# jkulhanek/viewformer

Hardware: NVIDIA H100
Metric: novel views/sec (128x128, 9-ctx) (higher is better)
Workload: dtype f32 encoder (bit-exact codes) + bf16 transformer/decoder

## Files before the change

viewformer_b200/csrc/vf_tc_gemm.cu:

```cuda
#include "vf_wgmma.cuh"
#include <stdlib.h>

namespace {
using namespace vftc;

constexpr int BLOCK_M = 128;
constexpr int ROW_BYTES = 128;
constexpr int A_STAGE_BYTES = BLOCK_M * ROW_BYTES;
constexpr int NUM_EPI_WARPS = 8;
constexpr int NUM_MMA_THREADS = 32 * NUM_EPI_WARPS;
constexpr int NUM_THREADS = NUM_MMA_THREADS + 128;

struct TcParams {
    CUtensorMap tmA, tmB;
    int conv;
    int M, Ncols;
    int num_k_blocks;
    int batch2;
    int tiles_m, tiles_n, total_tiles;
    int a_bm1, a_bm2, b_bm1, b_bm2;
    int TW, TH, TN, tiles_x, tiles_y, OH, OW, Nimg, cin_blocks, bk_elems;
    int tap_dy[9], tap_dx[9], tap_coff[9];
    int gemm_koff;
    int causal_block, causal_skip_n;
    float alpha;
    const float* bias;
    int bias_mode, act;
    const float* residual;
    float* C_f32;
    __nv_bfloat16* C_bf16;
    long long ldc, c_sb1, c_sb2;
    int vec_ok;
    int halo;
    double* gn_sums;
    int gn_groups, gn_cpg, gn_rows_per_img;
    int exact;
    int exact_kc;
    int exact_clog;
    int exact_kpp;
    int exact_lo_b;
    const float2* norm_mr;
    const float* norm_gamma;
    const float* norm_beta;
    int norm_groups, norm_cpg, norm_swish;
};

constexpr float EXACT_LO_SCALE = 1.0f / 2048.0f;

struct TileInfo {
    int m0, n0, b1, b2, img0, oy0, ox0, nkb;
    bool skip;
};

__device__ __forceinline__ TileInfo decode_tile(const TcParams& p, int t, int block_n) {
    TileInfo ti;
    const int n_tile = t % p.tiles_n;
    const int r = t / p.tiles_n;
    const int m_tile = r % p.tiles_m;
    const int bz = r / p.tiles_m;
    ti.b1 = bz / p.batch2;
    ti.b2 = bz % p.batch2;
    ti.m0 = m_tile * BLOCK_M;
    ti.n0 = n_tile * block_n;
    ti.nkb = p.num_k_blocks;
    ti.skip = false;
    if (p.causal_block > 0) {
        const int lim = ((ti.m0 + BLOCK_M - 1) / p.causal_block + 1) * p.causal_block;
        if (p.causal_skip_n) {
            ti.skip = ti.n0 >= lim;
        } else {
            const int kb = (lim + p.bk_elems - 1) / p.bk_elems;
            if (kb < ti.nkb) ti.nkb = kb;
        }
    }
    ti.img0 = ti.oy0 = ti.ox0 = 0;
    if (p.conv) {
        const int tx = m_tile % p.tiles_x;
        const int q = m_tile / p.tiles_x;
        ti.img0 = (q / p.tiles_y) * p.TN;
        ti.oy0 = (q % p.tiles_y) * p.TH;
        ti.ox0 = tx * p.TW;
    }
    return ti;
}

constexpr int HALO_BYTES = 23552;
constexpr int HALO_SLOTS = 6;
__host__ __device__ constexpr int operand_bytes(int stages, int stage_bytes, int b_stage_bytes) {
    return stages * stage_bytes > 2 * HALO_BYTES + HALO_SLOTS * b_stage_bytes ? stages * stage_bytes
                                                                               : 2 * HALO_BYTES + HALO_SLOTS * b_stage_bytes;
}
constexpr int MAX_STAGES = 8;
template <int kBlockN, int kStages>
__host__ __device__ constexpr int tc_smem_bytes() {
    return operand_bytes(kStages, A_STAGE_BYTES + kBlockN * ROW_BYTES, kBlockN * ROW_BYTES) +
           NUM_EPI_WARPS * 32 * (kBlockN / 2 + 4) * 4  + 1024  + 8 * (2 * MAX_STAGES + 4) ;
}

__device__ __forceinline__ void normalise_halo(const TcParams& p, uint8_t* tile, int cb, int img, int oy0, int ox0, int tid) {
    const int rows = (p.TW + 2) * (p.TH + 2);
    for (int idx = tid; idx < rows * 8; idx += NUM_MMA_THREADS) {
        const int r = idx >> 3, pc = idx & 7;
        const int py = r / (p.TW + 2), px = r - py * (p.TW + 2);
        const int iy = oy0 - 1 + py, ix = ox0 - 1 + px;
        if (iy < 0 || iy >= p.OH || ix < 0 || ix >= p.OW) continue;
        const int c0 = cb * 64 + ((pc ^ (r & 7)) << 3);
        uint4* ptr = reinterpret_cast<uint4*>(tile + r * ROW_BYTES + pc * 16);
        const uint4 v = *ptr;
        uint32_t w[4] = {v.x, v.y, v.z, v.w};
#pragma unroll
        for (int k = 0; k < 4; ++k) {
            const int c = c0 + 2 * k;
            const float2 ma = __ldg(p.norm_mr + (img * p.norm_groups + c / p.norm_cpg));
            const float2 mb = __ldg(p.norm_mr + (img * p.norm_groups + (c + 1) / p.norm_cpg));
            const float sa = ma.y * __ldg(p.norm_gamma + c), sb = mb.y * __ldg(p.norm_gamma + c + 1);
            float a = __uint_as_float(w[k] << 16), b = __uint_as_float(w[k] & 0xffff0000u);
            a = fmaf(a, sa, __ldg(p.norm_beta + c) - ma.x * sa);
            b = fmaf(b, sb, __ldg(p.norm_beta + c + 1) - mb.x * sb);
            if (p.norm_swish == 1) {
                a = __fdividef(a, 1.0f + __expf(-a));
                b = __fdividef(b, 1.0f + __expf(-b));
            }
            __nv_bfloat162 o = __floats2bfloat162_rn(a, b);
            w[k] = *reinterpret_cast<uint32_t*>(&o);
            if (p.norm_swish == 2) {
                uint32_t h, th;
                asm("mul.rn.bf16x2 %0, %1, %2;" : "=r"(h) : "r"(w[k]), "r"(0x3f003f00u));
                asm("tanh.approx.bf16x2 %0, %1;" : "=r"(th) : "r"(h));
                asm("fma.rn.bf16x2 %0, %1, %2, %1;" : "=r"(w[k]) : "r"(h), "r"(th));
            }
        }
        *ptr = make_uint4(w[0], w[1], w[2], w[3]);
    }
}

template <int kBlockN, int kStages, WgKind kKind>
__global__ void __launch_bounds__(NUM_THREADS, 1) tc_gemm_kernel(const __grid_constant__ TcParams p) {
    constexpr int B_STAGE_BYTES = kBlockN * ROW_BYTES;
    constexpr int STAGE_BYTES = A_STAGE_BYTES + B_STAGE_BYTES;
    constexpr int K_STEPS = 4;
    constexpr int HALF_N = kBlockN / 2;
    constexpr int STG_LD = HALF_N + 4;
    constexpr int STG_BYTES = NUM_EPI_WARPS * 32 * STG_LD * 4;
    constexpr int NACC = kBlockN / 2;
    constexpr bool kExact = kKind == F16;

    extern __shared__ uint8_t smem_raw[];
    uint8_t* smem = reinterpret_cast<uint8_t*>((reinterpret_cast<uintptr_t>(smem_raw) + 1023) & ~(uintptr_t)1023);
    constexpr int OPER_BYTES = operand_bytes(kStages, STAGE_BYTES, B_STAGE_BYTES);
    float* staging = reinterpret_cast<float*>(smem + OPER_BYTES);
    uint64_t* full_bar = reinterpret_cast<uint64_t*>(smem + OPER_BYTES + STG_BYTES);
    uint64_t* empty_bar = full_bar + MAX_STAGES;
    uint64_t* a_full_bar = empty_bar + MAX_STAGES;
    uint64_t* a_empty_bar = a_full_bar + 2;
    constexpr int NG = kStages;
    constexpr int NGH = HALO_SLOTS;
    uint8_t* halo_b_base = smem + 2 * HALO_BYTES;

    const int warp = threadIdx.x >> 5;
    const int lane = threadIdx.x & 31;

    if (threadIdx.x == 0) {
        prefetch_tmap(&p.tmA);
        prefetch_tmap(&p.tmB);
        for (int s = 0; s < MAX_STAGES; ++s) {
            mbar_init(&full_bar[s], 1);
            mbar_init(&empty_bar[s], NUM_MMA_THREADS);
        }
        for (int a = 0; a < 2; ++a) {
            mbar_init(&a_full_bar[a], 1);
            mbar_init(&a_empty_bar[a], NUM_MMA_THREADS);
        }
        mbar_fence_init();
    }
    __syncthreads();

    if (warp >= NUM_EPI_WARPS) {
        setmaxnreg_dec<40>();
        if (warp == NUM_EPI_WARPS && elect_one()) {
            int stage = 0;
            uint32_t phase = 0;
            int ab = 0;
            uint32_t aphase = 0;
            for (int t = blockIdx.x; t < p.total_tiles; t += gridDim.x) {
                const TileInfo ti = decode_tile(p, t, kBlockN);
                if (ti.skip) continue;
                if (p.halo) {
                    const uint32_t halo_bytes = (uint32_t)((p.TW + 2) * (p.TH + 2)) * ROW_BYTES;
                    const int nkb = 9 * p.cin_blocks;
                    int tap = 0, cb = 0;
                    for (int kb = 0; kb < nkb; ++kb) {
                        mbar_wait(&empty_bar[stage], phase ^ 1, "vf_tc_gemm producer");
                        mbar_expect_tx(&full_bar[stage], (uint32_t)B_STAGE_BYTES);
                        if (tap == 0) {
                            mbar_wait(&a_empty_bar[ab], aphase ^ 1, "vf_tc_gemm producer(halo)");
                            mbar_expect_tx(&a_full_bar[ab], halo_bytes);
                            tma_load_4d(smem + ab * HALO_BYTES, &p.tmA, &a_full_bar[ab], cb * p.bk_elems, ti.ox0 - 1, ti.oy0 - 1, ti.img0);
                            if (++ab == 2) { ab = 0; aphase ^= 1; }
                        }
                        tma_load_4d(halo_b_base + stage * B_STAGE_BYTES, &p.tmB, &full_bar[stage], (tap * p.cin_blocks + cb) * p.bk_elems,
                                    ti.n0, 0, 0);
                        if (++tap == 9) { tap = 0; ++cb; }
                        if (++stage == NGH) { stage = 0; phase ^= 1; }
                    }
                    continue;
                }
                for (int kb = 0; kb < ti.nkb; ++kb) {
                    mbar_wait(&empty_bar[stage], phase ^ 1, "vf_tc_gemm producer");
                    mbar_expect_tx(&full_bar[stage], (uint32_t)STAGE_BYTES);
                    uint8_t* sa = smem + stage * STAGE_BYTES;
                    uint8_t* sb = sa + A_STAGE_BYTES;
                    int kcoord_b = kb * p.bk_elems;
                    if (p.conv) {
                        int kbr = kb, a_half = 0;
                        if (p.exact) {
                            const int j = kb / p.exact_kpp;
                            kbr = kb - j * p.exact_kpp;
                            a_half = (j == 0) ? p.exact_clog : 0;
                            const int tap_ = kbr / p.cin_blocks, cb_ = kbr - tap_ * p.cin_blocks;
                            kcoord_b = ((tap_ * 2 + (j == 1 ? 1 : 0)) * p.cin_blocks + cb_) * p.bk_elems;
                        }
                        const int tap = kbr / p.cin_blocks;
                        const int cb = kbr - tap * p.cin_blocks;
                        tma_load_4d(sa, &p.tmA, &full_bar[stage], a_half + p.tap_coff[tap] + cb * p.bk_elems, ti.ox0 + p.tap_dx[tap],
                                    ti.oy0 + p.tap_dy[tap], ti.img0);
                    } else {
                        int kcoord_a = kb * p.bk_elems;
                        if (p.exact) {
                            const int j = kb / p.exact_kpp, kbr = kb - j * p.exact_kpp;
                            kcoord_a = (j == 0 ? p.exact_clog : 0) + kbr * p.bk_elems;
                            kcoord_b = (j == 1 ? p.exact_lo_b : 0) + kbr * p.bk_elems;
                        }
                        if (p.gemm_koff) kcoord_a += p.tap_coff[ti.b1];
                        tma_load_4d(sa, &p.tmA, &full_bar[stage], kcoord_a, ti.m0, ti.b2 * p.a_bm2, ti.b1 * p.a_bm1);
                    }
                    tma_load_4d(sb, &p.tmB, &full_bar[stage], kcoord_b, ti.n0, ti.b2 * p.b_bm2, ti.b1 * p.b_bm1);
                    if (++stage == NG) { stage = 0; phase ^= 1; }
                }
            }
        }
        return;
    }

    setmaxnreg_inc<232>();
    const int wg = warp >> 2;
    const int quarter = warp & 3;
    const int col_half = warp >> 2;
    float* stg = staging + warp * (32 * STG_LD);
    int stage = 0, ab = 0;
    uint32_t phase = 0, aphase = 0;

    auto to_staging = [&](const float (&v)[NACC], float sc) {
        const int r_lo = 64 * wg + 16 * (warp & 3) + (lane >> 2);
#pragma unroll
        for (int j = 0; j < NACC / 4; ++j) {
#pragma unroll
            for (int h = 0; h < 2; ++h) {
                const int r = r_lo + 8 * h, c = 8 * j + 2 * (lane & 3);
                float* dst = staging + ((c / HALF_N) * 4 + (r >> 5)) * (32 * STG_LD) + (r & 31) * STG_LD + (c % HALF_N);
                *reinterpret_cast<float2*>(dst) = make_float2(v[4 * j + 2 * h] * sc, v[4 * j + 2 * h + 1] * sc);
            }
        }
    };

    for (int t = blockIdx.x; t < p.total_tiles; t += gridDim.x) {
        const TileInfo ti = decode_tile(p, t, kBlockN);
        if (ti.skip) continue;

        float acc[NACC];
        float csum[kExact ? NACC : 1];
        auto k_loop = [&]() {
            const int nkb = p.halo ? 9 * p.cin_blocks : ti.nkb;
            const int nsmall = p.exact ? 2 * p.exact_kpp / p.exact_kc : 0;
            int prev_stage = -1, prev_halo = -1, in_chunk = 0, ck = 0, tap = 0;
            bool fresh = true;
            uint32_t a_base = 0;
            const uint32_t pitch = (uint32_t)(p.TW + 2);
            auto retire_prev = [&]() {
                if (prev_stage >= 0) mbar_arrive(&empty_bar[prev_stage]);
                if (prev_halo >= 0) mbar_arrive(&a_empty_bar[prev_halo]);
                prev_stage = prev_halo = -1;
            };
#pragma unroll 1
            for (int kb = 0; kb < nkb; ++kb) {
                uint64_t adesc, bdesc;
                const int this_halo = (p.halo && tap == 8) ? ab : -1;
                if (p.halo) {
                    if (tap == 0) {
                        mbar_wait(&a_full_bar[ab], aphase, "vf_tc_gemm mma(halo)");
                        a_base = smem_u32(smem + ab * HALO_BYTES);
                        if (!kExact && p.norm_mr) {
                            normalise_halo(p, smem + ab * HALO_BYTES, kb / 9, ti.img0, ti.oy0, ti.ox0, threadIdx.x);
                            fence_async_smem();
                            named_sync(1, NUM_MMA_THREADS);
                        }
                    }
                    mbar_wait(&full_bar[stage], phase, "vf_tc_gemm mma");
                    const uint32_t a_addr = a_base + ((uint32_t)(tap / 3) * pitch + (uint32_t)(tap % 3) + (uint32_t)(8 * wg) * pitch) * ROW_BYTES;
                    adesc = sw128_desc(a_addr, pitch * ROW_BYTES);
                    bdesc = sw128_desc(smem_u32(halo_b_base + stage * B_STAGE_BYTES));
                } else {
                    mbar_wait(&full_bar[stage], phase, "vf_tc_gemm mma");
                    const uint32_t sa = smem_u32(smem + stage * STAGE_BYTES);
                    adesc = sw128_desc(sa + (uint32_t)(wg * 64 * ROW_BYTES));
                    bdesc = sw128_desc(sa + A_STAGE_BYTES);
                }
                wgmma_fence();
#pragma unroll
                for (int k = 0; k < K_STEPS; ++k)
                    wgmma_ss<kBlockN, kKind>(acc, adesc + (uint64_t)(2 * k), bdesc + (uint64_t)(2 * k), (fresh && k == 0) ? 0u : 1u);
                wgmma_commit();
                fresh = false;
                wgmma_wait<1>();
                retire_prev();
                prev_stage = stage;
                prev_halo = this_halo;
                if (p.halo) {
                    if (++stage == NGH) { stage = 0; phase ^= 1; }
                    if (++tap == 9) { tap = 0; if (++ab == 2) { ab = 0; aphase ^= 1; } }
                } else {
                    if (++stage == NG) { stage = 0; phase ^= 1; }
                }
                if (kExact && ++in_chunk == p.exact_kc) {
                    in_chunk = 0;
                    wgmma_wait<0>();
                    reg_fence(acc);
                    const float sc = (ck < nsmall ? EXACT_LO_SCALE : 1.0f) * p.alpha;
                    if (ck == 0) {
#pragma unroll
                        for (int i = 0; i < NACC; ++i) csum[i] = acc[i] * sc;
                    } else {
#pragma unroll
                        for (int i = 0; i < NACC; ++i) csum[i] = fmaf(acc[i], sc, csum[i]);
                    }
                    ++ck;
                    fresh = true;
                }
            }
            wgmma_wait<0>();
            reg_fence(acc);
            retire_prev();
        };
        if constexpr (kExact) k_loop();

        const int row = quarter * 32 + lane;
        long long my_off;
        int my_ok, gm;
        if (p.conv) {
            const int lx = row % p.TW;
            const int q = row / p.TW;
            const int ly = q % p.TH;
            const int ln = q / p.TH;
            const int img = ti.img0 + ln, oy = ti.oy0 + ly, ox = ti.ox0 + lx;
            my_ok = (img < p.Nimg) && (oy < p.OH) && (ox < p.OW);
            gm = (img * p.OH + oy) * p.OW + ox;
            my_off = (long long)gm * p.ldc;
        } else {
            gm = ti.m0 + row;
            my_ok = gm < p.M;
            my_off = (long long)ti.b1 * p.c_sb1 + (long long)ti.b2 * p.c_sb2 + (long long)gm * p.ldc;
        }
        const float bias_m = (p.bias_mode == VF_BIAS_M && my_ok) ? __ldg(p.bias + gm) : 0.f;

        constexpr int VPR = HALF_N / 4;
        constexpr int RPI = 32 / VPR;
        constexpr int ITERS = 32 / RPI;
        const int r_sub = lane / VPR;
        const int c_ln = (lane % VPR) * 4;
        const int n_ln = ti.n0 + col_half * HALF_N + c_ln;
        const bool fast = p.vec_ok && (ti.n0 + kBlockN <= p.Ncols);
        auto residual_at = [&](int i) {
            const int rr = i * RPI + r_sub;
            const int ok = __shfl_sync(0xffffffffu, my_ok, rr);
            const long long off_row = __shfl_sync(0xffffffffu, my_off, rr);
            const long long o = ok ? off_row + n_ln : (long long)n_ln;
            return __ldg(reinterpret_cast<const float4*>(p.residual + o));
        };
        float4 resv[kExact ? 1 : ITERS];
        if (!kExact && fast && p.residual) {
#pragma unroll
            for (int i = 0; i < ITERS; ++i) resv[i] = residual_at(i);
        }
        float4 bias4 = make_float4(0.f, 0.f, 0.f, 0.f);
        if (fast && p.bias_mode == VF_BIAS_N) bias4 = __ldg(reinterpret_cast<const float4*>(p.bias + n_ln));

        if constexpr (!kExact) k_loop();
        named_sync(1, NUM_MMA_THREADS);
        if constexpr (kExact) to_staging(csum, 1.0f);
        else to_staging(acc, p.alpha);
        named_sync(1, NUM_MMA_THREADS);

        if (fast) {
            float gs = 0.f, gq = 0.f;
#pragma unroll
            for (int i = 0; i < ITERS; ++i) {
                const int rr = i * RPI + r_sub;
                const int ok = __shfl_sync(0xffffffffu, my_ok, rr);
                const long long off_row = __shfl_sync(0xffffffffu, my_off, rr);
                const float bm = __shfl_sync(0xffffffffu, bias_m, rr);
                float4 v = *reinterpret_cast<const float4*>(stg + rr * STG_LD + c_ln);
                if (p.bias_mode == VF_BIAS_N) { v.x += bias4.x; v.y += bias4.y; v.z += bias4.z; v.w += bias4.w; }
                else { v.x += bm; v.y += bm; v.z += bm; v.w += bm; }
                if (p.act == VF_ACT_GELU_ERF) { v.x = vf_gelu_erf(v.x); v.y = vf_gelu_erf(v.y); v.z = vf_gelu_erf(v.z); v.w = vf_gelu_erf(v.w); }
                if (p.residual) {
                    const float4 r = kExact ? residual_at(i) : resv[i];
                    v.x += r.x; v.y += r.y; v.z += r.z; v.w += r.w;
                }
                if (ok) {
                    gs += (v.x + v.y) + (v.z + v.w);
                    gq += (v.x * v.x + v.y * v.y) + (v.z * v.z + v.w * v.w);
                    const long long off = off_row + n_ln;
                    if (p.C_f32) *reinterpret_cast<float4*>(p.C_f32 + off) = v;
                    if (p.C_bf16) {
                        __nv_bfloat162 lo = __floats2bfloat162_rn(v.x, v.y), hi = __floats2bfloat162_rn(v.z, v.w);
                        uint2 u;
                        u.x = *reinterpret_cast<uint32_t*>(&lo);
                        u.y = *reinterpret_cast<uint32_t*>(&hi);
                        *reinterpret_cast<uint2*>(p.C_bf16 + off) = u;
                    }
                }
            }
            if (p.gn_sums) {
                const unsigned okmask = __ballot_sync(0xffffffffu, my_ok);
#pragma unroll
                for (int o = VPR; o < 32; o <<= 1) {
                    gs += __shfl_xor_sync(0xffffffffu, gs, o);
                    gq += __shfl_xor_sync(0xffffffffu, gq, o);
                }
                const int lpg = p.gn_cpg >> 2;
                for (int o = 1; o < lpg; o <<= 1) {
                    gs += __shfl_xor_sync(0xffffffffu, gs, o);
                    gq += __shfl_xor_sync(0xffffffffu, gq, o);
                }
                const int gm_first = __shfl_sync(0xffffffffu, gm, okmask ? (__ffs(okmask) - 1) : 0);
                if (okmask && r_sub == 0 && (lane % lpg) == 0) {
                    const long long slot = ((long long)(gm_first / p.gn_rows_per_img) * p.gn_groups + n_ln / p.gn_cpg) * 2;
                    atomicAdd(p.gn_sums + slot, (double)gs);
                    atomicAdd(p.gn_sums + slot + 1, (double)gq);
                }
            }
        } else {
#pragma unroll 1
            for (int rr = 0; rr < 32; ++rr) {
                const int ok = __shfl_sync(0xffffffffu, my_ok, rr);
                const long long off_row = __shfl_sync(0xffffffffu, my_off, rr);
                const float bm = __shfl_sync(0xffffffffu, bias_m, rr);
                if (!ok) continue;
                for (int c = lane; c < HALF_N; c += 32) {
                    const int n = ti.n0 + col_half * HALF_N + c;
                    if (n >= p.Ncols) continue;
                    float x = stg[rr * STG_LD + c];
                    x += (p.bias_mode == VF_BIAS_N) ? __ldg(p.bias + n) : bm;
                    if (p.act == VF_ACT_GELU_ERF) x = vf_gelu_erf(x);
                    const long long off = off_row + n;
                    if (p.residual) x += __ldg(p.residual + off);
                    if (p.C_f32) p.C_f32[off] = x;
                    if (p.C_bf16) p.C_bf16[off] = __float2bfloat16(x);
                }
            }
        }
    }
}

int make_tmap(CUtensorMap* tm, int dtype, const void* base, const uint64_t dims[4], const uint64_t strides_bytes[3],
              const uint32_t box[4]) {
    EncodeTiledFn fn = encode_fn();
    if (!fn) { vf_set_error("vf_tc_gemm: cuTensorMapEncodeTiled unavailable"); return VF_ERR_CUDA; }
    cuuint64_t gdim[4] = {dims[0], dims[1], dims[2], dims[3]};
    cuuint64_t gstr[3] = {strides_bytes[0], strides_bytes[1], strides_bytes[2]};
    cuuint32_t bx[4] = {box[0], box[1], box[2], box[3]};
    cuuint32_t es[4] = {1, 1, 1, 1};
    CUresult r = fn(tm, dtype == VF_BF16 ? CU_TENSOR_MAP_DATA_TYPE_BFLOAT16 : CU_TENSOR_MAP_DATA_TYPE_FLOAT32, 4,
                    const_cast<void*>(base), gdim, gstr, bx, es, CU_TENSOR_MAP_INTERLEAVE_NONE, CU_TENSOR_MAP_SWIZZLE_128B,
                    CU_TENSOR_MAP_L2_PROMOTION_L2_256B, CU_TENSOR_MAP_FLOAT_OOB_FILL_NONE);
    if (r != CUDA_SUCCESS) {
        vf_set_error("vf_tc_gemm: cuTensorMapEncodeTiled failed (%d): dims=[%llu,%llu,%llu,%llu] strides=[%llu,%llu,%llu] box=[%u,%u,%u,%u]",
                     (int)r, (unsigned long long)dims[0], (unsigned long long)dims[1], (unsigned long long)dims[2],
                     (unsigned long long)dims[3], (unsigned long long)strides_bytes[0], (unsigned long long)strides_bytes[1],
                     (unsigned long long)strides_bytes[2], box[0], box[1], box[2], box[3]);
        return VF_ERR_CUDA;
    }
    return VF_OK;
}

template <int kBlockN, int kStages, WgKind kKind>
int launch(const TcParams& prm, dim3 grid, cudaStream_t st) {
    constexpr int smem = tc_smem_bytes<kBlockN, kStages>();
    static_assert(kStages <= MAX_STAGES, "ring depth");
    static_assert(smem <= 232448, "shared memory budget");
    static vf_per_device_flag configured_pd;
    bool& configured = configured_pd.current();
    if (!configured) {
        cudaError_t e = cudaFuncSetAttribute(tc_gemm_kernel<kBlockN, kStages, kKind>, cudaFuncAttributeMaxDynamicSharedMemorySize, smem);
        if (e != cudaSuccess) { vf_set_error("vf_tc_gemm: cudaFuncSetAttribute: %s", cudaGetErrorString(e)); return VF_ERR_CUDA; }
        configured = true;
    }
    tc_gemm_kernel<kBlockN, kStages, kKind><<<grid, NUM_THREADS, smem, st>>>(prm);
    VF_CHECK_LAUNCH("vf_tc_gemm");
    return VF_OK;
}

template <int kBlockN, int kStages>
int launch_kind(const TcParams& prm, WgKind kind, dim3 grid, cudaStream_t st) {
    if (kind == TF32) return launch<kBlockN, kStages, TF32>(prm, grid, st);
    if (kind == F16) return launch<kBlockN, kStages, F16>(prm, grid, st);
    return launch<kBlockN, kStages, BF16>(prm, grid, st);
}

}

extern "C" int vf_tc_gemm(const vf_tc_gemm_t* q, vf_stream_t s) {
    VF_CHECK_ARG(q && q->A && q->B, "vf_tc_gemm: null operand");
    VF_CHECK_ARG(q->C_f32 || q->C_bf16, "vf_tc_gemm: no output");
    VF_CHECK_ARG(q->ab_dtype == VF_BF16 || q->ab_dtype == VF_F32 || q->ab_dtype == VF_F16X2, "vf_tc_gemm: bad dtype");
    const bool exact = q->ab_dtype == VF_F16X2;
    if (exact) {
        VF_CHECK_ARG(q->C_f32 && !q->C_bf16 && !q->norm_mean_rstd && q->causal_block == 0,
                     "vf_tc_gemm: VF_F16X2 (exact split-fp16) operands need an fp32 output and no causal / fused-norm options");
        if (q->conv) VF_CHECK_ARG(q->Ctot % 2 == 0 && q->alpha == 1.0f, "vf_tc_gemm: exact conv needs [hi | lo] channels and alpha = 1");
        else VF_CHECK_ARG(q->K % 64 == 0 && q->exact_lo_a >= q->K && q->exact_lo_b >= q->K && q->exact_lo_a % 8 == 0 && q->exact_lo_b % 8 == 0,
                          "vf_tc_gemm: exact GEMM needs K %% 64 == 0 and lo-half offsets >= K (K=%d lo_a=%lld lo_b=%lld)", q->K,
                          (long long)q->exact_lo_a, (long long)q->exact_lo_b);
    }
    VF_CHECK_ARG(q->bias_mode == VF_BIAS_NONE || q->bias, "vf_tc_gemm: bias pointer missing");
    VF_CHECK_ARG(!q->norm_mean_rstd || q->conv, "vf_tc_gemm: fused input GroupNorm is a convolution option");
    const bool tf32 = q->ab_dtype == VF_F32;
    const int tm_dtype = tf32 ? VF_F32 : VF_BF16;
    const int es = tf32 ? 4 : 2;
    const int bk = ROW_BYTES / es;

    TcParams prm;
    memset(&prm, 0, sizeof(prm));
    prm.conv = q->conv;
    prm.Ncols = q->Ncols;
    prm.bk_elems = bk;
    prm.alpha = q->alpha;
    prm.bias = q->bias;
    prm.bias_mode = q->bias_mode;
    prm.act = q->act;
    prm.residual = q->residual;
    prm.C_f32 = q->C_f32;
    prm.C_bf16 = reinterpret_cast<__nv_bfloat16*>(q->C_bf16);
    prm.ldc = q->ldc;
    prm.causal_block = q->causal_block;
    prm.causal_skip_n = q->causal_skip_n;

    const int block_n = (q->Ncols > 64) ? 128 : 64;
    const int b_box_rows = block_n;
    dim3 grid;
    int rc;
    if (q->conv) {
        VF_CHECK_ARG(q->ntaps >= 1 && q->ntaps <= 9, "vf_tc_gemm: ntaps");
        VF_CHECK_ARG(q->Cin % bk == 0 && q->Ctot % (16 / es) == 0, "vf_tc_gemm: conv Cin=%d must be a multiple of %d", q->Cin, bk);
        VF_CHECK_ARG(q->causal_block == 0, "vf_tc_gemm: causal with conv");
        int TW = q->OW >= 16 ? 16 : (q->OW >= 8 ? 8 : (q->OW >= 4 ? 4 : (q->OW >= 2 ? 2 : 1)));
        int TH = 128 / TW;
        if (TH > q->OH) { TH = 1; while (TH * 2 <= q->OH) TH *= 2; }
        int TN = 128 / (TW * TH);
        bool halo = !exact && q->ntaps == 9 && q->Ctot == q->Cin && q->OH == q->H && q->OW == q->W && q->OH >= 16 && q->OW >= 8;
        for (int t = 0; halo && t < 9; ++t) halo = q->tap_dy[t] == t / 3 - 1 && q->tap_dx[t] == t % 3 - 1 && q->tap_coff[t] == 0;
        if (halo) { TW = 8; TH = 16; TN = 1; }
        prm.halo = halo ? 1 : 0;
        if (q->norm_mean_rstd) {
            VF_CHECK_ARG(halo && q->ab_dtype == VF_BF16 && q->H >= 32 && q->Ncols % 128 == 0 && q->Cin % 64 == 0,
                         "vf_tc_gemm: fused input GroupNorm needs a 3x3 stride-1 bf16 conv on a map >= 32 rows (Cin %% 64 == 0, Cout %% 128 == 0)");
            VF_CHECK_ARG(q->norm_gamma && q->norm_beta && q->norm_groups > 0 && q->Cin % q->norm_groups == 0,
                         "vf_tc_gemm: fused input GroupNorm needs gamma, beta and a group count dividing Cin");
            prm.norm_mr = reinterpret_cast<const float2*>(q->norm_mean_rstd);
            prm.norm_gamma = q->norm_gamma;
            prm.norm_beta = q->norm_beta;
            prm.norm_groups = q->norm_groups;
            prm.norm_cpg = q->Cin / q->norm_groups;
            prm.norm_swish = q->norm_swish;
        }
        VF_CHECK_ARG(TW * TH * TN == 128 && TN <= 256, "vf_tc_gemm: cannot tile %dx%d output", q->OH, q->OW);
        prm.TW = TW; prm.TH = TH; prm.TN = TN;
        prm.tiles_x = (q->OW + TW - 1) / TW;
        prm.tiles_y = (q->OH + TH - 1) / TH;
        prm.OH = q->OH; prm.OW = q->OW; prm.Nimg = q->N;
        prm.cin_blocks = q->Cin / bk;
        prm.num_k_blocks = q->ntaps * prm.cin_blocks;
        if (exact) {
            prm.exact = 1;
            prm.exact_kpp = prm.num_k_blocks;
            prm.exact_clog = q->Ctot / 2;
            prm.exact_kc = (prm.num_k_blocks % 3 == 0) ? 3 : 1;
            prm.num_k_blocks *= 3;
        }
        prm.M = q->N * q->OH * q->OW;
        prm.batch2 = 1;
        for (int t = 0; t < q->ntaps; ++t) { prm.tap_dy[t] = q->tap_dy[t]; prm.tap_dx[t] = q->tap_dx[t]; prm.tap_coff[t] = q->tap_coff[t]; }
        const uint64_t dimsA[4] = {(uint64_t)q->Ctot, (uint64_t)q->W, (uint64_t)q->H, (uint64_t)q->N};
        const uint64_t strA[3] = {(uint64_t)q->Ctot * es, (uint64_t)q->W * q->Ctot * es, (uint64_t)q->H * q->W * q->Ctot * es};
        const uint32_t boxA[4] = {(uint32_t)bk, (uint32_t)(halo ? TW + 2 : TW), (uint32_t)(halo ? TH + 2 : TH), (uint32_t)TN};
        if ((rc = make_tmap(&prm.tmA, tm_dtype, q->A, dimsA, strA, boxA)) != VF_OK) return rc;
        const uint64_t Ktot = (uint64_t)q->ntaps * q->Cin * (exact ? 2 : 1);
        const uint64_t dimsB[4] = {Ktot, (uint64_t)q->Ncols, 1, 1};
        const uint64_t strB[3] = {Ktot * es, Ktot * es * q->Ncols, Ktot * es * q->Ncols};
        const uint32_t boxB[4] = {(uint32_t)bk, (uint32_t)b_box_rows, 1, 1};
        if ((rc = make_tmap(&prm.tmB, tm_dtype, q->B, dimsB, strB, boxB)) != VF_OK) return rc;
        const int ntiles_img = (q->N + TN - 1) / TN;
        grid = dim3(prm.tiles_x * prm.tiles_y * ntiles_img, (q->Ncols + block_n - 1) / block_n, 1);
    } else {
        VF_CHECK_ARG(q->M > 0 && q->Ncols > 0 && q->K > 0 && q->batch1 > 0 && q->batch2 > 0, "vf_tc_gemm: bad shape");
        VF_CHECK_ARG((q->lda * es) % 16 == 0 && (q->ldb * es) % 16 == 0, "vf_tc_gemm: row strides must be 16-byte multiples");
        VF_CHECK_ARG((q->a_sb1 * es) % 16 == 0 && (q->a_sb2 * es) % 16 == 0 && (q->b_sb1 * es) % 16 == 0 && (q->b_sb2 * es) % 16 == 0,
                     "vf_tc_gemm: batch strides must be 16-byte multiples");
        prm.M = q->M;
        prm.batch2 = q->batch2;
        prm.num_k_blocks = (q->K + bk - 1) / bk;
        if (exact) {
            prm.exact = 1;
            prm.exact_kpp = prm.num_k_blocks;
            prm.exact_clog = (int)q->exact_lo_a;
            prm.exact_lo_b = (int)q->exact_lo_b;
            prm.exact_kc = prm.exact_kpp % 4 == 0 ? 4 : (prm.exact_kpp % 3 == 0 ? 3 : (prm.exact_kpp % 2 == 0 ? 2 : 1));
            prm.num_k_blocks *= 3;
        }
        prm.c_sb1 = q->c_sb1; prm.c_sb2 = q->c_sb2;
        long long max_koff = 0;
        if (q->ntaps > 0) {
            VF_CHECK_ARG(q->ntaps == q->batch1 && q->ntaps <= 9, "vf_tc_gemm: gemm K offsets need ntaps == batch1 <= 9");
            prm.gemm_koff = 1;
            for (int t = 0; t < q->ntaps; ++t) {
                VF_CHECK_ARG(q->tap_coff[t] >= 0 && q->tap_coff[t] % 8 == 0, "vf_tc_gemm: K offsets must be non-negative multiples of 8 (16-byte TMA box starts)");
                prm.tap_coff[t] = q->tap_coff[t];
                if (q->tap_coff[t] > max_koff) max_koff = q->tap_coff[t];
            }
        }
        prm.a_bm1 = (q->batch1 > 1 && q->a_sb1 != 0) ? 1 : 0;
        prm.a_bm2 = (q->batch2 > 1 && q->a_sb2 != 0) ? 1 : 0;
        prm.b_bm1 = (q->batch1 > 1 && q->b_sb1 != 0) ? 1 : 0;
        prm.b_bm2 = (q->batch2 > 1 && q->b_sb2 != 0) ? 1 : 0;
        const uint64_t fbA = (uint64_t)q->lda * es * (uint64_t)q->M, fbB = (uint64_t)q->ldb * es * (uint64_t)q->Ncols;
        const uint64_t dimsA[4] = {(uint64_t)((exact ? q->exact_lo_a + q->K : q->K) + max_koff), (uint64_t)q->M, prm.a_bm2 ? (uint64_t)q->batch2 : 1, prm.a_bm1 ? (uint64_t)q->batch1 : 1};
        const uint64_t strA[3] = {(uint64_t)q->lda * es, prm.a_bm2 ? (uint64_t)q->a_sb2 * es : fbA, prm.a_bm1 ? (uint64_t)q->a_sb1 * es : fbA};
        const uint32_t boxA[4] = {(uint32_t)bk, (uint32_t)BLOCK_M, 1, 1};
        if ((rc = make_tmap(&prm.tmA, tm_dtype, q->A, dimsA, strA, boxA)) != VF_OK) return rc;
        const uint64_t dimsB[4] = {(uint64_t)(exact ? q->exact_lo_b + q->K : q->K), (uint64_t)q->Ncols, prm.b_bm2 ? (uint64_t)q->batch2 : 1, prm.b_bm1 ? (uint64_t)q->batch1 : 1};
        const uint64_t strB[3] = {(uint64_t)q->ldb * es, prm.b_bm2 ? (uint64_t)q->b_sb2 * es : fbB, prm.b_bm1 ? (uint64_t)q->b_sb1 * es : fbB};
        const uint32_t boxB[4] = {(uint32_t)bk, (uint32_t)b_box_rows, 1, 1};
        if ((rc = make_tmap(&prm.tmB, tm_dtype, q->B, dimsB, strB, boxB)) != VF_OK) return rc;
        VF_CHECK_ARG(q->causal_block == 0 || (q->causal_block % bk == 0 || bk % q->causal_block == 0), "vf_tc_gemm: causal block");
        grid = dim3((q->M + BLOCK_M - 1) / BLOCK_M, (q->Ncols + block_n - 1) / block_n, q->batch1 * q->batch2);
    }
    prm.tiles_m = (int)grid.x;
    prm.tiles_n = (int)grid.y;
    const long long total = (long long)prm.tiles_m * grid.y * grid.z;
    VF_CHECK_ARG(total > 0 && total < (1ll << 31), "vf_tc_gemm: tile count out of range");
    prm.total_tiles = (int)total;
    static int num_sms = 0;
    if (num_sms == 0) {
        int dev = 0;
        cudaGetDevice(&dev);
        if (cudaDeviceGetAttribute(&num_sms, cudaDevAttrMultiProcessorCount, dev) != cudaSuccess || num_sms <= 0) num_sms = 132;
    }
    const dim3 pgrid((unsigned)(total < num_sms ? total : num_sms), 1, 1);
    {
        auto a16 = [](const void* p) { return (reinterpret_cast<uintptr_t>(p) & 15) == 0; };
        auto a8 = [](const void* p) { return (reinterpret_cast<uintptr_t>(p) & 7) == 0; };
        prm.vec_ok = (q->ldc % 4 == 0) && (q->c_sb1 % 4 == 0) && (q->c_sb2 % 4 == 0) && a16(q->C_f32) && a8(q->C_bf16) && a16(q->residual) &&
                     a16(q->bias);
    }
    if (q->gn_sums) {
        const int C = q->Ncols;
        VF_CHECK_ARG(q->gn_groups > 0 && C % q->gn_groups == 0, "vf_tc_gemm: gn_groups");
        const int cpg = C / q->gn_groups;
        const long long rpi = q->conv ? (long long)q->OH * q->OW : q->gn_rows_per_img;
        const long long rows = q->conv ? (long long)q->N * q->OH * q->OW : (long long)q->M;
        VF_CHECK_ARG(cpg % 4 == 0 && cpg <= 32 && 32 % cpg == 0 && C % block_n == 0 && prm.vec_ok && rpi >= 32 && rpi % 32 == 0 &&
                         rows % rpi == 0 && (q->conv ? (prm.TW * prm.TH) % 32 == 0 : q->batch1 * q->batch2 == 1),
                     "vf_tc_gemm: fused GroupNorm statistics unsupported for this shape (C=%d groups=%d rows/img=%lld)", C, q->gn_groups, rpi);
        prm.gn_sums = q->gn_sums;
        prm.gn_groups = q->gn_groups;
        prm.gn_cpg = cpg;
        prm.gn_rows_per_img = (int)rpi;
        cudaError_t e = cudaMemsetAsync(q->gn_sums, 0, sizeof(double) * 2 * q->gn_groups * (rows / rpi), vf_s(s));
        if (e != cudaSuccess) { vf_set_error("vf_tc_gemm: memset gn_sums: %s", cudaGetErrorString(e)); return VF_ERR_CUDA; }
    }
    cudaStream_t st = vf_s(s);
    const WgKind kind = tf32 ? TF32 : (exact ? F16 : BF16);
    if (block_n == 128) return launch_kind<128, 4>(prm, kind, pgrid, st);
    return launch_kind<64, 6>(prm, kind, pgrid, st);
}
```

Measured before the change: 291.6.

## Use halo-tile TMA loads for exact split-precision conv and prefetch residual to L2

Extends the halo path, which loads one input tile with its border once and reuses it across all nine taps, to the exact (f16 hi/lo split) conv kernels. The halo buffers grow to four (two halves times two channel blocks), and B stages drop to four in that mode. The producer also issues bulk L2 prefetches of the residual rows, and the epilogue loads the residual in two batches instead of per-element. This cuts redundant per-tap A loads and residual latency, at the cost of more complex barrier phase tracking, a changed row mapping for TW=16, and a different shared-memory split.

```diff
diff --git a/viewformer_b200/csrc/vf_tc_gemm.cu b/viewformer_b200/csrc/vf_tc_gemm.cu
--- a/viewformer_b200/csrc/vf_tc_gemm.cu
+++ b/viewformer_b200/csrc/vf_tc_gemm.cu
@@ -85,16 +85,29 @@
 }
 
 constexpr int HALO_BYTES = 23552;
-constexpr int HALO_SLOTS = 6;
-__host__ __device__ constexpr int operand_bytes(int stages, int stage_bytes, int b_stage_bytes) {
-    return stages * stage_bytes > 2 * HALO_BYTES + HALO_SLOTS * b_stage_bytes ? stages * stage_bytes
-                                                                               : 2 * HALO_BYTES + HALO_SLOTS * b_stage_bytes;
+__host__ __device__ constexpr int halo_buffers(bool exact) { return exact ? 4 : 2; }
+__host__ __device__ constexpr int halo_slots(bool exact) { return exact ? 4 : 6; }
+__host__ __device__ constexpr int operand_bytes(int stages, int stage_bytes, int b_stage_bytes, bool exact) {
+    return stages * stage_bytes > halo_buffers(exact) * HALO_BYTES + halo_slots(exact) * b_stage_bytes
+               ? stages * stage_bytes
+               : halo_buffers(exact) * HALO_BYTES + halo_slots(exact) * b_stage_bytes;
 }
 constexpr int MAX_STAGES = 8;
-template <int kBlockN, int kStages>
+template <int kBlockN, int kStages, bool kExact>
 __host__ __device__ constexpr int tc_smem_bytes() {
-    return operand_bytes(kStages, A_STAGE_BYTES + kBlockN * ROW_BYTES, kBlockN * ROW_BYTES) +
-           NUM_EPI_WARPS * 32 * (kBlockN / 2 + 4) * 4  + 1024  + 8 * (2 * MAX_STAGES + 4) ;
+    return operand_bytes(kStages, A_STAGE_BYTES + kBlockN * ROW_BYTES, kBlockN * ROW_BYTES, kExact) +
+           NUM_EPI_WARPS * 32 * (kBlockN / 2 + 4) * 4  + 1024  + 8 * (2 * MAX_STAGES + 8) ;
+}
+
+__device__ __forceinline__ void prefetch_residual_l2(const TcParams& p, const TileInfo& ti, int block_n) {
+    const int tw = min(p.TW, p.OW - ti.ox0);
+    const uint32_t bytes = (uint32_t)(((long long)(tw - 1) * p.ldc + block_n) * 4);
+    for (int r = 0; r < p.TN * p.TH; ++r) {
+        const int img = ti.img0 + r / p.TH, oy = ti.oy0 + r % p.TH;
+        if (img >= p.Nimg || oy >= p.OH) continue;
+        const float* src = p.residual + ((long long)(img * p.OH + oy) * p.OW + ti.ox0) * p.ldc + ti.n0;
+        asm volatile("cp.async.bulk.prefetch.L2.global [%0], %1;" ::"l"(src), "r"(bytes) : "memory");
+    }
 }
 
 __device__ __forceinline__ void normalise_halo(const TcParams& p, uint8_t* tile, int cb, int img, int oy0, int ox0, int tid) {
@@ -147,15 +160,16 @@
 
     extern __shared__ uint8_t smem_raw[];
     uint8_t* smem = reinterpret_cast<uint8_t*>((reinterpret_cast<uintptr_t>(smem_raw) + 1023) & ~(uintptr_t)1023);
-    constexpr int OPER_BYTES = operand_bytes(kStages, STAGE_BYTES, B_STAGE_BYTES);
+    constexpr int OPER_BYTES = operand_bytes(kStages, STAGE_BYTES, B_STAGE_BYTES, kExact);
     float* staging = reinterpret_cast<float*>(smem + OPER_BYTES);
     uint64_t* full_bar = reinterpret_cast<uint64_t*>(smem + OPER_BYTES + STG_BYTES);
     uint64_t* empty_bar = full_bar + MAX_STAGES;
+    constexpr int NHB = halo_buffers(kExact);
     uint64_t* a_full_bar = empty_bar + MAX_STAGES;
-    uint64_t* a_empty_bar = a_full_bar + 2;
+    uint64_t* a_empty_bar = a_full_bar + NHB;
     constexpr int NG = kStages;
-    constexpr int NGH = HALO_SLOTS;
-    uint8_t* halo_b_base = smem + 2 * HALO_BYTES;
+    constexpr int NGH = halo_slots(kExact);
+    uint8_t* halo_b_base = smem + NHB * HALO_BYTES;
 
     const int warp = threadIdx.x >> 5;
     const int lane = threadIdx.x & 31;
@@ -167,7 +181,7 @@
             mbar_init(&full_bar[s], 1);
             mbar_init(&empty_bar[s], NUM_MMA_THREADS);
         }
-        for (int a = 0; a < 2; ++a) {
+        for (int a = 0; a < NHB; ++a) {
             mbar_init(&a_full_bar[a], 1);
             mbar_init(&a_empty_bar[a], NUM_MMA_THREADS);
         }
@@ -181,12 +195,36 @@
             int stage = 0;
             uint32_t phase = 0;
             int ab = 0;
-            uint32_t aphase = 0;
-            for (int t = blockIdx.x; t < p.total_tiles; t += gridDim.x) {
+            uint32_t aphase = 0, tpar = 0;
+            for (int t = blockIdx.x; t < p.total_tiles; t += gridDim.x, tpar ^= 1) {
                 const TileInfo ti = decode_tile(p, t, kBlockN);
                 if (ti.skip) continue;
+                const uint32_t halo_bytes = (uint32_t)((p.TW + 2) * (p.TH + 2)) * ROW_BYTES;
+                if (kExact && p.halo) {
+                    auto load_halves = [&](int h) {
+                        for (int cb = 0; cb < p.cin_blocks; ++cb) {
+                            const int hb = 2 * h + cb;
+                            mbar_wait(&a_empty_bar[hb], tpar ^ 1, "vf_tc_gemm producer(halo)");
+                            mbar_expect_tx(&a_full_bar[hb], halo_bytes);
+                            tma_load_4d(smem + hb * HALO_BYTES, &p.tmA, &a_full_bar[hb], (h ? 0 : p.exact_clog) + cb * p.bk_elems,
+                                        ti.ox0 - 1, ti.oy0 - 1, ti.img0);
+                        }
+                    };
+                    load_halves(0);
+                    if (p.residual && p.vec_ok && ti.n0 + kBlockN <= p.Ncols) prefetch_residual_l2(p, ti, kBlockN);
+                    int j = 0, tap = 0, cb = 0;
+                    for (int kb = 0; kb < ti.nkb; ++kb) {
+                        if (kb == NGH) load_halves(1);
+                        mbar_wait(&empty_bar[stage], phase ^ 1, "vf_tc_gemm producer");
+                        mbar_expect_tx(&full_bar[stage], (uint32_t)B_STAGE_BYTES);
+                        tma_load_4d(halo_b_base + stage * B_STAGE_BYTES, &p.tmB, &full_bar[stage],
+                                    ((tap * 2 + (j == 1 ? 1 : 0)) * p.cin_blocks + cb) * p.bk_elems, ti.n0, 0, 0);
+                        if (++cb == p.cin_blocks) { cb = 0; if (++tap == 9) { tap = 0; ++j; } }
+                        if (++stage == NGH) { stage = 0; phase ^= 1; }
+                    }
+                    continue;
+                }
                 if (p.halo) {
-                    const uint32_t halo_bytes = (uint32_t)((p.TW + 2) * (p.TH + 2)) * ROW_BYTES;
                     const int nkb = 9 * p.cin_blocks;
                     int tap = 0, cb = 0;
                     for (int kb = 0; kb < nkb; ++kb) {
@@ -205,6 +243,7 @@
                     }
                     continue;
                 }
+                if (kExact && p.conv && p.residual && p.vec_ok && ti.n0 + kBlockN <= p.Ncols) prefetch_residual_l2(p, ti, kBlockN);
                 for (int kb = 0; kb < ti.nkb; ++kb) {
                     mbar_wait(&empty_bar[stage], phase ^ 1, "vf_tc_gemm producer");
                     mbar_expect_tx(&full_bar[stage], (uint32_t)STAGE_BYTES);
@@ -248,34 +287,37 @@
     const int col_half = warp >> 2;
     float* stg = staging + warp * (32 * STG_LD);
     int stage = 0, ab = 0;
-    uint32_t phase = 0, aphase = 0;
-
+    uint32_t phase = 0, aphase = 0, tpar = 0;
+
+    const bool col_split = kExact && p.halo && p.TW == 16;
     auto to_staging = [&](const float (&v)[NACC], float sc) {
         const int r_lo = 64 * wg + 16 * (warp & 3) + (lane >> 2);
 #pragma unroll
         for (int j = 0; j < NACC / 4; ++j) {
 #pragma unroll
             for (int h = 0; h < 2; ++h) {
-                const int r = r_lo + 8 * h, c = 8 * j + 2 * (lane & 3);
+                const int r = col_split ? 16 * (2 * (warp & 3) + h) + 8 * wg + (lane >> 2) : r_lo + 8 * h;
+                const int c = 8 * j + 2 * (lane & 3);
                 float* dst = staging + ((c / HALF_N) * 4 + (r >> 5)) * (32 * STG_LD) + (r & 31) * STG_LD + (c % HALF_N);
                 *reinterpret_cast<float2*>(dst) = make_float2(v[4 * j + 2 * h] * sc, v[4 * j + 2 * h + 1] * sc);
             }
         }
     };
 
-    for (int t = blockIdx.x; t < p.total_tiles; t += gridDim.x) {
+    for (int t = blockIdx.x; t < p.total_tiles; t += gridDim.x, tpar ^= 1) {
         const TileInfo ti = decode_tile(p, t, kBlockN);
         if (ti.skip) continue;
 
         float acc[NACC];
         float csum[kExact ? NACC : 1];
         auto k_loop = [&]() {
-            const int nkb = p.halo ? 9 * p.cin_blocks : ti.nkb;
+            const int nkb = (p.halo && !kExact) ? 9 * p.cin_blocks : ti.nkb;
             const int nsmall = p.exact ? 2 * p.exact_kpp / p.exact_kc : 0;
-            int prev_stage = -1, prev_halo = -1, in_chunk = 0, ck = 0, tap = 0;
+            int prev_stage = -1, prev_halo = -1, in_chunk = 0, ck = 0, tap = 0, j = 0, cb = 0;
             bool fresh = true;
             uint32_t a_base = 0;
             const uint32_t pitch = (uint32_t)(p.TW + 2);
+            const uint32_t wg_rows = p.TW == 16 ? 8u : 8u * pitch;
             auto retire_prev = [&]() {
                 if (prev_stage >= 0) mbar_arrive(&empty_bar[prev_stage]);
                 if (prev_halo >= 0) mbar_arrive(&a_empty_bar[prev_halo]);
@@ -284,8 +326,17 @@
 #pragma unroll 1
             for (int kb = 0; kb < nkb; ++kb) {
                 uint64_t adesc, bdesc;
-                const int this_halo = (p.halo && tap == 8) ? ab : -1;
-                if (p.halo) {
+                int this_halo = (p.halo && tap == 8) ? ab : -1;
+                if (kExact && p.halo) {
+                    const int hb = (j == 0 ? 0 : 2) + cb;
+                    if (tap == 0 && j < 2) mbar_wait(&a_full_bar[hb], tpar, "vf_tc_gemm mma(halo)");
+                    this_halo = (tap == 8 && j != 1) ? hb : -1;
+                    mbar_wait(&full_bar[stage], phase, "vf_tc_gemm mma");
+                    const uint32_t a_addr = smem_u32(smem + hb * HALO_BYTES) +
+                                            ((uint32_t)(tap / 3) * pitch + (uint32_t)(tap % 3) + (uint32_t)wg * wg_rows) * ROW_BYTES;
+                    adesc = sw128_desc(a_addr, pitch * ROW_BYTES);
+                    bdesc = sw128_desc(smem_u32(halo_b_base + stage * B_STAGE_BYTES));
+                } else if (p.halo) {
                     if (tap == 0) {
                         mbar_wait(&a_full_bar[ab], aphase, "vf_tc_gemm mma(halo)");
                         a_base = smem_u32(smem + ab * HALO_BYTES);
@@ -315,7 +366,10 @@
                 retire_prev();
                 prev_stage = stage;
                 prev_halo = this_halo;
-                if (p.halo) {
+                if (kExact && p.halo) {
+                    if (++stage == NGH) { stage = 0; phase ^= 1; }
+                    if (++cb == p.cin_blocks) { cb = 0; if (++tap == 9) { tap = 0; ++j; } }
+                } else if (p.halo) {
                     if (++stage == NGH) { stage = 0; phase ^= 1; }
                     if (++tap == 9) { tap = 0; if (++ab == 2) { ab = 0; aphase ^= 1; } }
                 } else {
@@ -376,11 +430,15 @@
             const long long o = ok ? off_row + n_ln : (long long)n_ln;
             return __ldg(reinterpret_cast<const float4*>(p.residual + o));
         };
-        float4 resv[kExact ? 1 : ITERS];
-        if (!kExact && fast && p.residual) {
-#pragma unroll
-            for (int i = 0; i < ITERS; ++i) resv[i] = residual_at(i);
-        }
+        constexpr int RB = kExact ? ITERS / 2 : ITERS;
+        float4 resv[RB];
+        auto load_residual = [&](int i0) {
+            if (fast && p.residual) {
+#pragma unroll
+                for (int i = 0; i < RB; ++i) resv[i] = residual_at(i0 + i);
+            }
+        };
+        if constexpr (!kExact) load_residual(0);
         float4 bias4 = make_float4(0.f, 0.f, 0.f, 0.f);
         if (fast && p.bias_mode == VF_BIAS_N) bias4 = __ldg(reinterpret_cast<const float4*>(p.bias + n_ln));
 
@@ -394,6 +452,7 @@
             float gs = 0.f, gq = 0.f;
 #pragma unroll
             for (int i = 0; i < ITERS; ++i) {
+                if (kExact && i % RB == 0) load_residual(i);
                 const int rr = i * RPI + r_sub;
                 const int ok = __shfl_sync(0xffffffffu, my_ok, rr);
                 const long long off_row = __shfl_sync(0xffffffffu, my_off, rr);
@@ -403,7 +462,7 @@
                 else { v.x += bm; v.y += bm; v.z += bm; v.w += bm; }
                 if (p.act == VF_ACT_GELU_ERF) { v.x = vf_gelu_erf(v.x); v.y = vf_gelu_erf(v.y); v.z = vf_gelu_erf(v.z); v.w = vf_gelu_erf(v.w); }
                 if (p.residual) {
-                    const float4 r = kExact ? residual_at(i) : resv[i];
+                    const float4 r = resv[i % RB];
                     v.x += r.x; v.y += r.y; v.z += r.z; v.w += r.w;
                 }
                 if (ok) {
@@ -485,7 +544,7 @@
 
 template <int kBlockN, int kStages, WgKind kKind>
 int launch(const TcParams& prm, dim3 grid, cudaStream_t st) {
-    constexpr int smem = tc_smem_bytes<kBlockN, kStages>();
+    constexpr int smem = tc_smem_bytes<kBlockN, kStages, kKind == F16>();
     static_assert(kStages <= MAX_STAGES, "ring depth");
     static_assert(smem <= 232448, "shared memory budget");
     static vf_per_device_flag configured_pd;
@@ -557,9 +616,11 @@
         int TH = 128 / TW;
         if (TH > q->OH) { TH = 1; while (TH * 2 <= q->OH) TH *= 2; }
         int TN = 128 / (TW * TH);
-        bool halo = !exact && q->ntaps == 9 && q->Ctot == q->Cin && q->OH == q->H && q->OW == q->W && q->OH >= 16 && q->OW >= 8;
+        bool halo = q->ntaps == 9 && q->OH == q->H && q->OW == q->W &&
+                    (exact ? q->Ctot == 2 * q->Cin && q->Cin <= 2 * bk && TN == 1 && TW >= 8
+                           : q->Ctot == q->Cin && q->OH >= 16 && q->OW >= 8);
         for (int t = 0; halo && t < 9; ++t) halo = q->tap_dy[t] == t / 3 - 1 && q->tap_dx[t] == t % 3 - 1 && q->tap_coff[t] == 0;
-        if (halo) { TW = 8; TH = 16; TN = 1; }
+        if (halo && !exact) { TW = 8; TH = 16; TN = 1; }
         prm.halo = halo ? 1 : 0;
         if (q->norm_mean_rstd) {
             VF_CHECK_ARG(halo && q->ab_dtype == VF_BF16 && q->H >= 32 && q->Ncols % 128 == 0 && q->Cin % 64 == 0,
```

After: 317.3 (median of 6 runs). 1.09x the previous value.
